# xl-tang3/RCOT

Hardware: AMD Instinct MI355X
Metric: 128x128 patches/sec (gen+critic step) (higher is better)
Workload: dtype fp32 (exact fp32 MFMA everywhere); 1 GPU; BASELINE configs[1]: Restormer T_net(decoder=True)+F_net(128), denoise_50, RMSprop, paired, B=8/GPU 128x128; global_batch=8, patch=128, parallelism=dp1, gemm_prec=fp32

## Files before the change

### include/rcot_hip.h

```cpp
#ifndef RCOT_HIP_H
#define RCOT_HIP_H
#include <stddef.h>

#ifdef __cplusplus
extern "C" {
#endif

#define RCOT_ABI_VERSION 26

#define RCOT_PREC_FP32 0
#define RCOT_PREC_BF16X3 1
#define RCOT_PREC_BF16X6 2
#define RCOT_PREC_BF16X1 3

int rcot_abi_version(void);
int rcot_debug_nt_coop(int mask);
int rcot_profile_begin(void);
int rcot_profile_end(char* out, int n);
int rcot_last_kernel(char* out, int n);

int rcot_conv1x1_fwd(const float* W, long ldw, const float* X, long sXb, float* Y, long sYb, int B, int Ci, int Co,
                     int N, const float* ln_mu, const float* ln_rs, const float* ln_w, const float* ln_b,
                     const float* R, long sRb, float beta, void* stream);
int rcot_conv1x1_dgrad(const float* W, long ldw, const float* dY, long sdYb, float* dX, long sdXb, int B, int Ci,
                       int Co, int N, float beta, void* stream);
int rcot_conv1x1_wgrad(const float* dY, long sdYb, const float* X, long sXb, float* dW, long ldw, int B, int Ci,
                       int Co, int N, const float* ln_mu, const float* ln_rs, const float* ln_w, const float* ln_b,
                       float beta, float* ws, size_t ws_bytes, int prec, void* stream);
int rcot_conv1x1_wgrad_slabs(const float* dY, long sdYb, const float* X, long sXb, int B, int Ci, int Co, int N,
                             const float* ln_mu, const float* ln_rs, const float* ln_w, const float* ln_b, float* ws,
                             size_t ws_bytes, int prec, int* S, int* ldws, void* stream);
// ... 47 lines not shown
int rcot_conv2d_dgrad(const float* dY, const float* Wt, float* dX, int B, int Ci, int H, int W, int Co, int KH,
                      int KW, int stride, int pad, float beta, const float* mask, float mslope, float* ws, size_t ws_bytes,
                      void* stream);
int rcot_conv2d_wgrad(const float* dY, const float* X, float* dWt, int B, int Ci, int H, int W, int Co, int KH,
                      int KW, int stride, int pad, float beta, float* ws, size_t ws_bytes, void* stream);
int rcot_conv_pcm_prep(const float* X, float* out, long ldo, int B, int C, int H, int W, int mode, void* stream);
int rcot_conv_pcm_wgrad(const float* dZp, const float* Xp, long ld, int N, int Wp, int Co, int Ci, float* dW, float beta, float* ws,
                        size_t ws_bytes, int prec, void* stream);
int rcot_conv_pcm_merge(const float* dQ, long ldq, float* dX, int B, int C, int H, int W, void* stream);
int rcot_conv_pcm_pack(const float* W, const int* rowoff, const int* koff, int M, int K, void* Apk, void* stream);
int rcot_conv_pcm(const void* Apk, int M, int K, const float* Xp, long ldb, int N, const int* tapoff, int ntaps, const float* bias,
                  float lrelu, const int* colmap, float* Y, long ldy, float* ws, size_t ws_bytes, void* stream);
int rcot_pixel_shuffle(const float* in, float* out, long planes, int H, int W, int mode, void* stream);

int rcot_ln_stats(const float* x, float* mu, float* rs, int B, int C, int N, void* stream);
int rcot_ln_bwd(const float* g, const float* x, const float* mu, const float* rs, const float* w, const float* dres,
                float* dx, float* dw, float* db, int B, int C, int N, void* ws, long ws_bytes, void* stream);
int rcot_ln_bwd_rows(int B, int C, int N);
int rcot_block_param_reduce(const float* part1, const float* part2, int rows, int C, float* gw1, float* gb1, float* gw2,
                            float* gb2, const float* dWo_part, float* gWo, const float* dtemp_part, float* gtemp, int B,
                            int heads, const long long* slab_sets, int n_sets, void* stream);

int rcot_dwconv3x3(const float* x, const float* w, float* y, int B, int C, int H, int W, int flip, void* stream);
int rcot_gdfn_gate_fwd(const float* p, const float* w, float* g, int B, int hid, int H, int W, void* stream);
int rcot_gdfn_gate_bwd(const float* p, const float* w, const float* dg, float* dd, float* dwg, int B, int hid, int H,
                       int W, void* stream);
int rcot_gdfn_bwd(const float* p, const float* w, const float* dg, float* dp, float* dwg, float* dd_scratch, int B, int hid,
                  int H, int W, void* stream);
int rcot_dwconv3x3_wgrad(const float* dy, const float* x, float* dw, int B, int C, int H, int W, void* stream);
int rcot_dwconv3x3_bwd(const float* dy, const float* x, const float* w, float* dx, float* dwg, int B, int C, int H, int W,
                       void* stream);

int rcot_row_sumsq(const float* x, float* out, int B, int R, int N, long sXb, void* stream);
int rcot_attn_softmax(const float* Graw, int S, int ld, const float* sq, const float* temp, float* Gn, float* A, int B,
                      int heads, int c, void* stream);
int rcot_attn_bwd_small(const float* dA, const float* A, const float* Gn, const float* sq, const float* temp,
                        float* dtemp_part, float* Eq, float* EqT, float* Dq, float* Dk, int B, int heads, int c,
                        void* stream);
int rcot_attn_bwd_fused(const float* dM, const float* Wo, const float* A, const float* Gn, const float* sq, const float* temp,
                        float* Mf, float* dWo_part, float* dtemp_part, float* Eq, float* EqT, float* Dq, float* Dk, int B,
                        int heads, int c, void* ws, long ws_bytes, void* stream);
int rcot_attn_core_fwd(const float* u, long sUb, const float* temp, const float* WoT, long ldwt, float* sq, float* Gn, float* A,
                       float* MfT, long ldm, long sMb, int B, int heads, int c, int N, float* ws, size_t ws_bytes, void* stream);
int rcot_attn_core_bwd(const float* dM, int S, int ldd, const float* Wo, const float* A, const float* Gn, const float* sq,
                       const float* temp, float* Mf, float* dWo_part, float* dtemp_part, float* Eq, float* EqT, float* Dq, float* Dk, int B,
                       int heads, int c, void* stream);
int rcot_batch_reduce(const float* src, float* dst, int B, long n, float beta, void* stream);

int rcot_lrelu_bwd(const float* dy, const float* a, float* dz, long n, float slope, void* stream);
int rcot_bias_grad(const float* dz, float* db, int B, int C, int P, void* stream);
int rcot_axpby2d(const float* x, long sx, const float* y, long sy, float* out, long so, long rows, long cols, float a,
                 float b, void* stream);
int rcot_fill(float* p, long n, float v, void* stream);
int rcot_lerp(const float* t, const float* f, const float* alpha, float* out, int B, long per, void* stream);
int rcot_gp_penalty(const float* g, float* norms, float* u0, float* gp_out, int B, long per, float inv_global_batch,
                    void* stream);

int rcot_ot_reduce(const float* degraded, const float* restored, const float* target, float* sums, int B, long per,
                   void* stream);
int rcot_fft_plan(int n, int* radices, int cap);
int rcot_ot_spectrum(const float* degraded, const float* restored, const int* de_id, float* gF, float* spec, float* ws,
                     size_t ws_bytes, int B, int H, int W, void* stream);
int rcot_ot_grad(const float* degraded, const float* restored, const float* target, const int* de_id, const float* gF,
                 const float* sums, const float* spec, float* dout, float* scal, int B, long per, float sigma,
                 float Sigma, long global_batch, void* stream);

// ... 28 lines not shown
```

### rcot_amd/csrc/attn_core.hip

```cpp
#include <cstdlib>
#include "common.h"
#include "../../include/rcot_hip.h"

using namespace rcot;

namespace {

typedef float f32x4 __attribute__((ext_vector_type(4)));

__device__ __forceinline__ float clamp_norm(float sumsq) { return fmaxf(sqrtf(sumsq), 1e-12f); }

template <int CT>
struct AC {
    static constexpr int cp = 16 * CT;
    static constexpr int c = CT == 2 ? 24 : cp;
    static constexpr int LDA = (cp % 32 == 16) ? cp : cp + 16;
    static constexpr int PX = CT == 6 ? 128 : 256;
    static constexpr int Q4 = PX / 4;
    static constexpr int LDQ = PX + 8;
    static constexpr int NW = CT == 6 ? 8 : 4;
    static constexpr int NT = 64 * NW;
    static constexpr int RPP = NT / Q4;
    static constexpr int KQ = cp / RPP;
    static constexpr int MTW = CT == 6 ? 1 : 2;
// ... 254 lines not shown
                const int i = wave + NW * r, j = lane + 64 * q;
                a[r][q] += (i < c && j < c) ? gp[(long)s * cc + i * c + j] : 0.f;
            }
    }
#pragma unroll
    for (int r = 0; r < NR; ++r)
#pragma unroll
        for (int q = 0; q < NJ; ++q) {
            const int i = wave + NW * r, j = lane + 64 * q;
            if (i < c && j < c) Gs[i * LDA + j] = a[r][q];
        }
    const float* sp = sqpart + z * S * 2 * c;
    for (int r = tid; r < 2 * c; r += NT) {
        float t = sp[r];
        for (int s = 1; s < S; ++s) t += sp[(long)s * 2 * c + r];
        sqs[r < c ? r : cp + r - c] = t;
        if (ms == 0) sq[(long)b * 2 * C + (r < c ? h * c + r : C + h * c + r - c)] = t;
    }
    __syncthreads();
    attn_tail<CT>(Gs, sqs, bfr, h, b, heads, temp, Gn, A, MfT, ldm, sMb, mt0, mt1, ms == 0);
}

template <int CT>
int launch_core_fwd(const float* u, long sUb, const float* temp, const float* WoT, long ldwt, float* sq, float* Gn, float* A, float* MfT,
                    long ldm, long sMb, int B, int heads, int c, int N, float* ws, size_t ws_bytes, hipStream_t st) {
    using K = AC<CT>;
    const int C = heads * c;
    static bool once = (hipFuncSetAttribute((const void*)qk_stats_kernel<CT>, hipFuncAttributeMaxDynamicSharedMemorySize, 160 * 1024) ==
                        hipSuccess);
    (void)once;
    const int ms = cdiv(C / 16, K::MT_WG);
    if (N == 256 && CT != 6) {
        RCOT_LAUNCH(qk_stats_kernel<CT>, dim3(ms, heads, B), dim3(K::NT), K::smem_stats, st, u, sUb, heads, N, N, nullptr,
                           nullptr, temp, WoT, ldwt, sq, Gn, A, MfT, ldm, sMb);
        RCOT_LAUNCH_CHECK();
        return RCOT_OK;
    }
    const int pxw = N == 256 ? 128 : (N > 16384 && N % 2048 == 0) ? 2048 : ((N > 1024 && N % 512 == 0) ? 512 : 256);
    const int S = N / pxw;
    const size_t Z = (size_t)B * heads;
    const size_t need = Z * S * ((size_t)c * c + 2 * c) * sizeof(float);
    if (!ws || ws_bytes < need) return RCOT_EWORKSPACE;
    float* gpart = ws;
    float* sqpart = ws + Z * S * c * c;
    RCOT_LAUNCH(qk_stats_kernel<CT>, dim3(S, heads, B), dim3(K::NT), K::smem_stats, st, u, sUb, heads, N, pxw, gpart, sqpart,
                       temp, WoT, ldwt, sq, Gn, A, MfT, ldm, sMb);
// ... 246 lines not shown
    RCOT_LAUNCH_CHECK();
    return RCOT_OK;
}

}

extern "C" {

int rcot_attn_core_fwd(const float* u, long sUb, const float* temp, const float* WoT, long ldwt, float* sq, float* Gn, float* A,
                       float* MfT, long ldm, long sMb, int B, int heads, int c, int N, float* ws, size_t ws_bytes, void* stream) {
    if (!u || !temp || !WoT || !sq || !Gn || !A || !MfT || B <= 0 || heads <= 0 || c <= 0 || N <= 0 || B > 65535 || heads > 65535)
        return RCOT_EINVAL;
    const int C = heads * c;
    if ((reinterpret_cast<uintptr_t>(u) & 15) || (sUb & 3) || ldwt < C || ldm < C) return RCOT_EINVAL;
    if ((C % 16) || (N % 256) || N > 65536) return RCOT_EUNSUPPORTED;
    if (N > 4096 && (N % 512)) return RCOT_EUNSUPPORTED;
    hipStream_t st = (hipStream_t)stream;
    if (c == 48) return launch_core_fwd<3>(u, sUb, temp, WoT, ldwt, sq, Gn, A, MfT, ldm, sMb, B, heads, c, N, ws, ws_bytes, st);
    if (c == 96) return launch_core_fwd<6>(u, sUb, temp, WoT, ldwt, sq, Gn, A, MfT, ldm, sMb, B, heads, c, N, ws, ws_bytes, st);
    if (c == 24) return launch_core_fwd<2>(u, sUb, temp, WoT, ldwt, sq, Gn, A, MfT, ldm, sMb, B, heads, c, N, ws, ws_bytes, st);
    return RCOT_EUNSUPPORTED;
}

int rcot_attn_core_bwd(const float* dM, int S, int ldd, const float* Wo, const float* A, const float* Gn, const float* sq,
                       const float* temp, float* Mf, float* dWo_part, float* dtemp_part, float* Eq, float* EqT, float* Dq, float* Dk, int B,
                       int heads, int c, void* stream) {
    if (!dM || !Wo || !A || !Gn || !sq || !temp || !Mf || !dWo_part || !dtemp_part || !Eq || !EqT || !Dq || !Dk || B <= 0 ||
        heads <= 0 || B > 65535 || heads > 65535 || S < 0 || S > 8)
        return RCOT_EINVAL;
    const int C = heads * c;
    if ((C % 16) || (c != 24 && c != 48 && c != 96)) return RCOT_EUNSUPPORTED;
    if (S == 0) ldd = C;
    if (ldd < C || (ldd & 3) || (reinterpret_cast<uintptr_t>(dM) & 15) || (reinterpret_cast<uintptr_t>(Wo) & 15)) return RCOT_EINVAL;
    const long sDs = (long)C * ldd, sDb = (long)(S < 1 ? 1 : S) * sDs;
    hipStream_t st = (hipStream_t)stream;
    if (c == 48) return launch_core_bwd<3>(dM, S, ldd, sDs, sDb, Wo, A, Gn, sq, temp, Mf, dWo_part, dtemp_part, Eq, EqT, Dq, Dk, B, heads, st);
    if (c == 96) return launch_core_bwd<6>(dM, S, ldd, sDs, sDb, Wo, A, Gn, sq, temp, Mf, dWo_part, dtemp_part, Eq, EqT, Dq, Dk, B, heads, st);
    return launch_core_bwd<2>(dM, S, ldd, sDs, sDb, Wo, A, Gn, sq, temp, Mf, dWo_part, dtemp_part, Eq, EqT, Dq, Dk, B, heads, st);
}

}
```

### rcot_amd/csrc/pointwise.hip

```cpp
#include <cstdlib>
#include "common.h"
#include "../../include/rcot_hip.h"

using namespace rcot;

namespace {

constexpr int LN_TX = 16, LN_TY = 16, LN_PIX = LN_TX * 4;

__device__ __forceinline__ float4 f4_add(float4 a, float4 b) { return make_float4(a.x + b.x, a.y + b.y, a.z + b.z, a.w + b.w); }

template <int TX>
__device__ __forceinline__ float4 reduce_rows(float4 v, float4* red, int tx, int ty) {
    constexpr int TY = 256 / TX;
    __syncthreads();
    red[ty * TX + tx] = v;
    __syncthreads();
    float4 t = red[tx];
#pragma unroll
    for (int i = 1; i < TY; ++i) t = f4_add(t, red[i * TX + tx]);
    return t;
}

__global__ __launch_bounds__(256) void ln_stats_kernel(const float* __restrict__ x, float* __restrict__ mu,
// ... 431 lines not shown
    b.plane = q / ((long)hq * wq);
    const int rem = (int)(q - b.plane * (long)hq * wq);
    const int ys = rem / wq;
    b.y0 = ys * 4;
    b.x0 = (rem - ys * wq) * 4;
    return b;
}

template <bool FLIP, bool NB>
__global__ __launch_bounds__(256) void dwconv_kernel(const float* __restrict__ x, const float* __restrict__ w,
                                                     float* __restrict__ y, long nblocks, int C, int H, int W) {
    const long q = (long)blockIdx.x * 256 + threadIdx.x;
    if (q >= nblocks) return;
    const BlockIdx4 b = block4(q, H, W);
    const int c = (int)(b.plane % C);
    Patch r;
    if (NB) load_patch_nb(x + b.plane * H * W, H, W, b.y0, b.x0, r);
    else load_patch(x + b.plane * H * W, H, W, b.y0, b.x0, r);
    float o[4][4];
    stencil16<FLIP>(r, w + c * 9, o);
    float* yp = y + b.plane * H * W + (long)b.y0 * W + b.x0;
#pragma unroll
    for (int i = 0; i < 4; ++i) *reinterpret_cast<float4*>(yp + (long)i * W) = make_float4(o[i][0], o[i][1], o[i][2], o[i][3]);
}

template <bool NB>
__global__ __launch_bounds__(256) void gate_fwd_kernel(const float* __restrict__ p, const float* __restrict__ w,
                                                       float* __restrict__ g, long nblocks, int hid, int H, int W) {
    const long q = (long)blockIdx.x * 256 + threadIdx.x;
    if (q >= nblocks) return;
    const BlockIdx4 b = block4(q, H, W);
    const long bi = b.plane / hid;
    const int j = (int)(b.plane - bi * hid);
    const long hw = (long)H * W;
    const float* p1 = p + (bi * 2 * hid + j) * hw;
    Patch r;
    float d1[4][4], d2[4][4];
    if (NB) {
        PatchRows q1, q2;
        patch_request(p1, H, W, b.y0, b.x0, q1);
        patch_request(p1 + (long)hid * hw, H, W, b.y0, b.x0, q2);
        patch_land(q1, H, W, b.y0, b.x0, r);
        stencil16<false>(r, w + j * 9, d1);
        patch_land(q2, H, W, b.y0, b.x0, r);
        stencil16<false>(r, w + (j + hid) * 9, d2);
    } else {
// ... 739 lines not shown
    RCOT_LAUNCH_CHECK();
    return RCOT_OK;
}

int rcot_dwconv3x3(const float* x, const float* w, float* y, int B, int C, int H, int W, int flip, void* stream) {
    if (!x || !w || !y || B <= 0 || C <= 0 || H <= 0 || W <= 0) return RCOT_EINVAL;
    if ((W & 3) || (H & 3)) {
        if (flip) return RCOT_EINVAL;
        const long total = (long)B * C * H * W;
        RCOT_LAUNCH(dwconv_any_kernel, dim3(grid_for(total)), dim3(256), 0, (hipStream_t)stream, x, w, y, total, C, H, W);
        RCOT_LAUNCH_CHECK();
        return RCOT_OK;
    }
    const long nq = (long)B * C * (H >> 2) * (W >> 2);
    const bool nb = nb_lanes_ok(W);
#define RCOT_DW(F, NB_) do { note_kernel("dwconv_kernel<%s, %s>", tf(F), tf(NB_)); RCOT_LAUNCH((dwconv_kernel<F, NB_>), dim3(cdiv(nq, 256)), dim3(256), 0, (hipStream_t)stream, x, w, y, nq, C, H, W); } while (0)
    if (flip) { if (nb) RCOT_DW(true, true); else RCOT_DW(true, false); }
    else { if (nb) RCOT_DW(false, true); else RCOT_DW(false, false); }
#undef RCOT_DW
    RCOT_LAUNCH_CHECK();
    return RCOT_OK;
}

int rcot_gdfn_gate_fwd(const float* p, const float* w, float* g, int B, int hid, int H, int W, void* stream) {
    if (!p || !w || !g || B <= 0 || hid <= 0 || H <= 0 || W <= 0) return RCOT_EINVAL;
    if ((W & 3) || (H & 3)) {
        const long total = (long)B * hid * H * W;
        RCOT_LAUNCH(gate_fwd_any_kernel, dim3(grid_for(total)), dim3(256), 0, (hipStream_t)stream, p, w, g, total, hid, H, W);
        RCOT_LAUNCH_CHECK();
        return RCOT_OK;
    }
    const long nq = (long)B * hid * (H >> 2) * (W >> 2);
    if (nb_lanes_ok(W))
        RCOT_LAUNCH(gate_fwd_kernel<true>, dim3(cdiv(nq, 256)), dim3(256), 0, (hipStream_t)stream, p, w, g, nq, hid, H, W);
    else
        RCOT_LAUNCH(gate_fwd_kernel<false>, dim3(cdiv(nq, 256)), dim3(256), 0, (hipStream_t)stream, p, w, g, nq, hid, H, W);
    RCOT_LAUNCH_CHECK();
    return RCOT_OK;
}

int rcot_gdfn_gate_bwd(const float* p, const float* w, const float* dg, float* dd, float* dwg, int B, int hid, int H,
                       int W, void* stream) {
    if (!p || !w || !dg || !dd || B <= 0 || hid <= 0 || H <= 0 || W <= 0 || (W & 3) || (H & 3)) return RCOT_EINVAL;
    const long cols = (long)B * hid * (W >> 2);
    bool fused = true;
    int rc;
// ... 128 lines not shown
```

### rcot_amd/lib.py

```python
from __future__ import annotations

import ctypes as C
import os

_HERE = os.path.dirname(os.path.abspath(__file__))
ABI_VERSION = 26
PREC_FP32, PREC_BF16X3, PREC_BF16X6, PREC_BF16X1 = 0, 1, 2, 3
LIB_PATH = os.environ.get("RCOT_LIB") or os.path.join(_HERE, "librcot_hip.so")


class RcotLibraryError(RuntimeError):
    pass


class RcotKernelError(RuntimeError):
    pass


_f = C.c_void_p
_l = C.c_long
_i = C.c_int
_fl = C.c_float
_d = C.c_double
_sz = C.c_size_t

class KmajorDesc(C.Structure):
    _fields_ = [("At", _f), ("lda", _l), ("sAo", _l), ("sAi", _l), ("a_rows", _i),
                ("Bm", _f), ("ldb", _l), ("sBo", _l), ("sBi", _l),
                ("C", _f), ("ldc", _l), ("sCo", _l), ("sCi", _l),
# ... 21 lines not shown
                         _f, _f, _l, _i, _f, _f, _f, _f, _f, _i, _i, _i, _i, _i, _fl, _f, _sz, _i, _f],
    "rcot_gemm_kmajor_stats": [_f, _l, _l, _l, _i, _f, _l, _l, _l, _f, _l, _l, _l, _f, _l, _l, _l, _f, _f, _l, _i, _i, _i, _i, _i, _f],
    "rcot_kmajor_desc_size": [],
    "rcot_gemm_kmajor_multi": [_f, _i, _i, _i, _f],
    "rcot_pack_weight": [_f, _l, _i, _i, _f, _f, _f, _f, _f, _f, _f, _f, _f, _f, _f, _f, _f],
    "rcot_pack_weights": [_f, _f, _i, _f],
    "rcot_linear_fwd": [_f, _f, _f, _f, _i, _i, _i, _fl, _f, _sz, _f],
    "rcot_linear_dgrad": [_f, _f, _f, _i, _i, _i, _f, _sz, _f],
    "rcot_linear_wgrad": [_f, _f, _f, _i, _i, _i, _fl, _f],
    "rcot_conv2d_fwd": [_f, _f, _f, _f, _i, _i, _i, _i, _i, _i, _i, _i, _i, _fl, _i, _f, _f, _fl, _f, _sz, _f],
    "rcot_conv2d_dgrad": [_f, _f, _f, _i, _i, _i, _i, _i, _i, _i, _i, _i, _fl, _f, _fl, _f, _sz, _f],
    "rcot_conv2d_wgrad": [_f, _f, _f, _i, _i, _i, _i, _i, _i, _i, _i, _i, _fl, _f, _sz, _f],
    "rcot_conv_pcm_prep": [_f, _f, _l, _i, _i, _i, _i, _i, _f],
    "rcot_conv_pcm_wgrad": [_f, _f, _l, _i, _i, _i, _i, _f, _fl, _f, _sz, _i, _f],
    "rcot_conv_pcm_merge": [_f, _l, _f, _i, _i, _i, _i, _f],
    "rcot_conv_pcm_pack": [_f, _f, _f, _i, _i, _f, _f],
    "rcot_conv_pcm": [_f, _i, _i, _f, _l, _i, _f, _i, _f, _fl, _f, _f, _l, _f, _sz, _f],
    "rcot_pixel_shuffle": [_f, _f, _l, _i, _i, _i, _f],
    "rcot_ln_stats": [_f, _f, _f, _i, _i, _i, _f],
    "rcot_ln_bwd": [_f, _f, _f, _f, _f, _f, _f, _f, _f, _i, _i, _i, _f, _l, _f],
    "rcot_ln_bwd_rows": [_i, _i, _i],
    "rcot_block_param_reduce": [_f, _f, _i, _i, _f, _f, _f, _f, _f, _f, _f, _f, _i, _i, _f, _i, _f],
    "rcot_dwconv3x3": [_f, _f, _f, _i, _i, _i, _i, _i, _f],
    "rcot_gdfn_gate_fwd": [_f, _f, _f, _i, _i, _i, _i, _f],
    "rcot_gdfn_gate_bwd": [_f, _f, _f, _f, _f, _i, _i, _i, _i, _f],
    "rcot_gdfn_bwd": [_f, _f, _f, _f, _f, _f, _i, _i, _i, _i, _f],
    "rcot_dwconv3x3_wgrad": [_f, _f, _f, _i, _i, _i, _i, _f],
    "rcot_dwconv3x3_bwd": [_f, _f, _f, _f, _f, _i, _i, _i, _i, _f],
    "rcot_row_sumsq": [_f, _f, _i, _i, _i, _l, _f],
    "rcot_attn_softmax": [_f, _i, _i, _f, _f, _f, _f, _i, _i, _i, _f],
    "rcot_attn_bwd_small": [_f, _f, _f, _f, _f, _f, _f, _f, _f, _f, _i, _i, _i, _f],
    "rcot_attn_bwd_fused": [_f] * 13 + [_i, _i, _i, _f, _l, _f],
    "rcot_attn_core_fwd": [_f, _l, _f, _f, _l, _f, _f, _f, _f, _l, _l, _i, _i, _i, _i, _f, _sz, _f],
    "rcot_attn_core_bwd": [_f, _i, _i] + [_f] * 12 + [_i, _i, _i, _f],
    "rcot_batch_reduce": [_f, _f, _i, _l, _fl, _f],
    "rcot_lrelu_bwd": [_f, _f, _f, _l, _fl, _f],
    "rcot_bias_grad": [_f, _f, _i, _i, _i, _f],
    "rcot_axpby2d": [_f, _l, _f, _l, _f, _l, _l, _l, _fl, _fl, _f],
    "rcot_fill": [_f, _l, _fl, _f],
    "rcot_lerp": [_f, _f, _f, _f, _i, _l, _f],
    "rcot_gp_penalty": [_f, _f, _f, _f, _i, _l, _fl, _f],
    "rcot_ot_reduce": [_f, _f, _f, _f, _i, _l, _f],
    "rcot_fft_plan": [_i, _f, _i],
    "rcot_ot_spectrum": [_f, _f, _f, _f, _f, _f, _sz, _i, _i, _i, _f],
    "rcot_ot_grad": [_f, _f, _f, _f, _f, _f, _f, _f, _f, _i, _l, _fl, _fl, _l, _f],
    "rcot_patch_prep": [_f, _f, _i, _i, _i, _i, _i, _i, _fl, C.c_ulonglong, _f, _f, _f],
    "rcot_rmsprop_step": [_f, _f, _f, _l, _d, _d, _d, _d, _f],
    "rcot_adam_step": [_f, _f, _f, _f, _l, _d, _d, _d, _d, _i, _d, _f],
    "rcot_prelu_fwd": [_f, _f, _f, _l, _f],
    "rcot_prelu_bwd": [_f, _f, _f, _f, _f, _l, _f, _sz, _f],
    "rcot_row_dot": [_f, _f, _f, _l, _i, _fl, _f],
    "rcot_row_scale_add": [_f, _f, _f, _f, _fl, _f, _l, _i, _f],
    "rcot_ca_gate_fwd": [_f, _f, _f, _f, _f, _i, _i, _i, _f],
    "rcot_ca_gate_bwd": [_f, _f, _f, _f, _f, _f, _f, _f, _f, _i, _i, _i, _f, _sz, _f],
    "rcot_bilinear_down2": [_f, _f, _l, _i, _i, _f],
    "rcot_bilinear_down2_bwd": [_f, _f, _l, _i, _i, _fl, _f],
# ... 48 lines not shown
```

### rcot_amd/net_restormer.py

```python
from __future__ import annotations

from collections import OrderedDict
from typing import Callable, Dict, List, Optional

import numpy as np

import torch

from . import params as P


class ParamStore:

    def __init__(self, be, shapes, live_order: List[str], dead: List[str]):
        self.be = be
        self.shapes = list(shapes)
        self.layout = P.make_layout(shapes, live_order, dead)
        self.flat = be.zeros(self.layout.n_total)
        self.grad = be.zeros(self.layout.n_total)
        self.p: Dict[str, torch.Tensor] = {}
        self.g: Dict[str, torch.Tensor] = {}
        for name, shp in self.shapes:
            o = self.layout.offset[name]
            n = int(np.prod(shp))
# ... 120 lines not shown
        B, C3, H, W = u.shape
        N = H * W
        uu = u.view(B, 3, self.heads, self.c, N)
        return uu[:, 0], uu[:, 1], u.view(B, 3, self.C, N)[:, 2].unsqueeze(1)

    def forward(self, x, save: bool, wmask: Optional[int] = None, in_stats=None, want_stats: bool = False):
        assert not (save and wmask is not None)
        be, C, hd, c, hid = self.be, self.C, self.heads, self.c, self.hid
        B, _, H, W = x.shape
        N = H * W
        fast = be.kmajor_worth(C, N, B)
        pstats = wmask is None and getattr(be, "stats_ok", None) is not None and be.stats_ok(C, N, B)
        self.out_stats = None
        t = be.empty(B, 3 * C, H, W)
        if in_stats is not None and pstats:
            mu1, rs1 = in_stats
            be.conv1x1_fwd(self.Wqkv, x, t, ln=(mu1, rs1, self.w1, self.b1), packed=self.pk_qkv)
        else:
            mu1, rs1 = be.empty(B, N), be.empty(B, N)
            be.conv1x1_fwd(self.Wqkv, x, t, ln=(mu1, rs1, self.w1, self.b1), packed=self.pk_qkv, ln_compute=True)
        if wmask is not None:
            t[..., wmask:].zero_()
        u = be.empty(B, 3 * C, H, W)
        be.dwconv3x3(t, self.Wdw, u)
        if wmask is not None:
            u[..., wmask:].zero_()
        sq = be.empty(B, 2 * C)
        Q, K, V = self._qkv_views(u)
        Gn, A, MfT = be.empty(B, hd, c, c), be.empty(B, hd, c, c), be.empty(B, C, C)
        if not be.attn_core_fwd(u, self.temp, self.pk_o[0], sq, Gn, A, MfT):
            be.row_sumsq(u[:, :2 * C], sq)
            Graw = be.bmm_nt_slabs(Q, K)
            if Graw is None:
                Graw = be.empty(B, hd, c, c)
                be.bmm_nt(Q, K, Graw)
            be.attn_softmax(Graw, sq, self.temp, Gn, A)
            be.bmm_nn(A, self._woT_heads(B), MfT.view(B, hd, c, C), transA=True)
        y = be.empty(B, C, H, W)
        mu2, rs2 = be.empty(B, N), be.empty(B, N)
        if fast and pstats:
            be.gemm_kmajor_stats(MfT.unsqueeze(1), V, y.view(B, 1, C, N), C, C, x.view(B, 1, C, N), (mu2, rs2))
        elif fast:
            be.gemm_kmajor(MfT.unsqueeze(1), V, y.view(B, 1, C, N), C, C, R=x.view(B, 1, C, N))
        else:
            be.bmm_nn(MfT.unsqueeze(1), V, y.view(B, 1, C, N), transA=True, R=x.view(B, 1, C, N))
        pp = be.empty(B, 2 * hid, H, W)
        be.conv1x1_fwd(self.Win, y, pp, ln=(mu2, rs2, self.w2, self.b2), packed=self.pk_in, ln_compute=not (fast and pstats))
        if wmask is not None:
            pp[..., wmask:].zero_()
        gg = be.empty(B, hid, H, W)
        be.gdfn_gate_fwd(pp, self.Wdw2, gg)
        out = be.empty(B, C, H, W)
        if want_stats and pstats and fast:
            self.out_stats = (be.empty(B, N), be.empty(B, N))
            be.conv1x1_fwd(self.Wout, gg, out, R=y, packed=self.pk_out, stats=self.out_stats)
        else:
            be.conv1x1_fwd(self.Wout, gg, out, R=y, packed=self.pk_out)
        ctx = (x, mu1, rs1, t, u, sq, Gn, A, y, mu2, rs2, pp, gg) if save else None
        return out, ctx

# ... 676 lines not shown
```

### rcot_amd/ops.py

```python
from __future__ import annotations

from typing import Optional, Sequence, Tuple

import os
import sys

import ctypes as C

import torch

from . import lib as _lib

LN = Optional[Tuple[torch.Tensor, torch.Tensor, torch.Tensor, torch.Tensor]]


ctypes_ll = C.c_longlong


def _ptr(t: Optional[torch.Tensor]):
    return None if t is None else t.data_ptr()


_raw_stream = getattr(torch._C, "_cuda_getCurrentRawStream", None) or (lambda i: torch.cuda.current_stream(i).cuda_stream)

# ... 58 lines not shown
    dev = torch.cuda.current_device() if torch.cuda.is_available() else -1
    if dev not in _DEFAULT:
        _DEFAULT[dev] = HipBackend()
    return _DEFAULT[dev]


class HipBackend:

    name = "hip"

    def __init__(self, device: Optional[torch.device] = None, workspace_bytes: int = 256 << 20):
        if not torch.cuda.is_available():
            raise _lib.RcotLibraryError("no HIP device visible: the RCOT hot path has no CPU fallback")
        self.L = _lib.load()
        self.device = torch.device("cuda", torch.cuda.current_device()) if device is None else torch.device(device)
        self._dev_index = self.device.index if self.device.index is not None else torch.cuda.current_device()
        self.ws = torch.empty(workspace_bytes // 4, dtype=torch.float32, device=self.device)
        self.ws_bytes = self.ws.numel() * 4
        self.prec = PREC_BY_NAME[os.environ.get("RCOT_GEMM_PREC", DEFAULT_PREC)]
        self._poison = os.environ.get("RCOT_POISON", "0") == "1"
        self.overlap = os.environ.get("RCOT_OVERLAP", "1") != "0"
        self._raw_events = os.environ.get("RCOT_RAW_EVENTS", "1") != "0"
        self.attn_core_maxn = 4096
        self.ln_fused = True
        self.prod_stats = True
        self._ev_ring, self._ev_next = [], -1
        self.x6_packs = self.prec == _lib.PREC_BF16X6
        self._side = torch.cuda.Stream(device=self.device) if self.overlap else None
        self._ws_side = torch.empty_like(self.ws) if self.overlap else None
        self._ws_slabs_gen = [torch.empty_like(self.ws), torch.empty_like(self.ws)]
        self._held = []
        self._pcm_cache = {}
        self._pcm_pinned = {}
        self._pcm_touched = set()
        self.pcm_pinning = False
        self._plan = None
        self._side_pending = False
        self._ln_scratch = [[torch.empty(1024 * 1024, dtype=torch.float32, device=self.device) for _ in range(2)] for _ in range(2)]
        self._ln_rows = 0
        self._gen = 0
        self._gen_event = [None, None]
        self._held_gen = [[], []]
        self._defer_close_env = os.environ.get("RCOT_DEFER_CLOSE")

    @property
    def defer_close(self):
# ... 703 lines not shown
                launch()
            if self._raw_events:
                ev, side = self._new_handover(), self._side.cuda_stream
                self._host(lambda: ev.record(side))
            else:
                ev = torch.cuda.Event()
                self._host(lambda: ev.record(self._side))
            self._gen_event[g] = ev
            self._held_gen[g] = self._held + [dWo_part, dtemp_part]
            self._held = []
            self._side_pending = True
            self._gen ^= 1
            return
        if close_block:
            self.side_join()
        launch()

    def dwconv3x3(self, x, w, y, flip: bool = False):
        B, Cc, H, W = x.shape
        assert x.is_contiguous() and y.is_contiguous() and w.is_contiguous()
        _lib.check(self.L.rcot_dwconv3x3(x.data_ptr(), w.data_ptr(), y.data_ptr(), B, Cc, H, W, int(flip), self._st()),
                   "rcot_dwconv3x3")

    def gdfn_gate_fwd(self, p, w, g):
        B, c2, H, W = p.shape
        assert p.is_contiguous() and g.is_contiguous() and w.is_contiguous()
        _lib.check(self.L.rcot_gdfn_gate_fwd(p.data_ptr(), w.data_ptr(), g.data_ptr(), B, c2 // 2, H, W, self._st()),
                   "rcot_gdfn_gate_fwd")

    def gdfn_gate_bwd(self, p, w, dg, dd, dw=None):
        B, c2, H, W = p.shape
        assert p.is_contiguous() and dg.is_contiguous() and dd.is_contiguous() and (dw is None or dw.is_contiguous())
        _lib.check(self.L.rcot_gdfn_gate_bwd(p.data_ptr(), w.data_ptr(), dg.data_ptr(), dd.data_ptr(), _ptr(dw), B, c2 // 2,
                                             H, W, self._st()), "rcot_gdfn_gate_bwd")

    @staticmethod
    def gdfn_bwd_needs_scratch(H: int, W: int) -> bool:
        wq = W // 4
        if wq > 64 or 64 % wq:
            return True
        for rs in (16, 8, 4):
            tpp = -(-H // rs) * wq
            if not (tpp % 256 == 0 or tpp % 64 == 0 or (tpp < 64 and tpp & (tpp - 1) == 0)):
                return True
        return False

# ... 12 lines not shown

    def dwconv3x3_wgrad(self, dy, x, dw):
        B, Cc, H, W = x.shape
        assert dy.is_contiguous() and x.is_contiguous() and dw.is_contiguous()
        _lib.check(self.L.rcot_dwconv3x3_wgrad(dy.data_ptr(), x.data_ptr(), dw.data_ptr(), B, Cc, H, W, self._st()),
                   "rcot_dwconv3x3_wgrad")

    def row_sumsq(self, x, out):
        B, R, N, sx = self._bcn(x, "row_sumsq x")
        assert out.is_contiguous()
        _lib.check(self.L.rcot_row_sumsq(x.data_ptr(), out.data_ptr(), B, R, N, sx, self._st()), "rcot_row_sumsq")

    def attn_softmax(self, Graw, sq, temp, Gn, A):
        B, heads, c, _ = Gn.shape
        for t in (sq, temp, Gn, A):
            assert t.is_contiguous()
        if isinstance(Graw, tuple):
            gp, S, ld = Graw
        else:
            assert Graw.is_contiguous() and tuple(Graw.shape) == tuple(Gn.shape)
            gp, S, ld = Graw.data_ptr(), 0, c
        _lib.check(self.L.rcot_attn_softmax(gp, S, ld, sq.data_ptr(), temp.data_ptr(), Gn.data_ptr(), A.data_ptr(),
                                            B, heads, c, self._st()), "rcot_attn_softmax")

    def attn_core_fwd(self, u, temp, WoT, sq, Gn, A, MfT) -> bool:
        B, heads, c, _ = Gn.shape
        N = u.shape[2] * u.shape[3]
        if N > self.attn_core_maxn:
            return False
        for t in (u, temp, sq, Gn, A, MfT):
            assert t.is_contiguous()
        assert WoT.stride(1) == 1 and tuple(MfT.shape) == (B, heads * c, heads * c) and u.shape[1] == 3 * heads * c
        rc = self.L.rcot_attn_core_fwd(u.data_ptr(), u.stride(0), temp.data_ptr(), WoT.data_ptr(), WoT.stride(0), sq.data_ptr(),
                                       Gn.data_ptr(), A.data_ptr(), MfT.data_ptr(), MfT.stride(1), MfT.stride(0), B, heads, c, N,
                                       self.ws.data_ptr(), self.ws_bytes, self._st())
        if rc == _lib.EUNSUPPORTED:
            return False
        _lib.check(rc, "rcot_attn_core_fwd")
        return True

    def attn_bwd_small(self, dA, A, Gn, sq, temp, dtemp_part, Eq, EqT, Dq, Dk):
        B, heads, c, _ = A.shape
        for t in (dA, A, Gn, sq, temp, dtemp_part, Eq, EqT, Dq, Dk):
            assert t.is_contiguous()
        _lib.check(self.L.rcot_attn_bwd_small(dA.data_ptr(), A.data_ptr(), Gn.data_ptr(), sq.data_ptr(), temp.data_ptr(),
                                              dtemp_part.data_ptr(), Eq.data_ptr(), EqT.data_ptr(), Dq.data_ptr(), Dk.data_ptr(), B, heads,
# ... 191 lines not shown
```

### rcot_amd/profiling.py

```python
from __future__ import annotations

import ctypes
from collections import defaultdict
from typing import Dict

import torch

GEMM_OPS = ("gemm_kmajor", "gemm_kmajor_stats", "gemm_kmajor_multi", "conv1x1_fwd", "conv1x1_dgrad", "conv1x1_dgrad_wgrad_slabs", "conv1x1_wgrad", "conv1x1_wgrad_slabs", "bmm_nn", "bmm_nt",
            "bmm_nt_slabs", "linear_fwd", "linear_dgrad",
            "linear_wgrad", "conv2d_fwd", "conv2d_dgrad", "conv2d_wgrad")
OTHER_OPS = ("ln_stats", "ln_bwd", "dwconv3x3", "gdfn_gate_fwd", "gdfn_gate_bwd", "gdfn_bwd", "dwconv3x3_wgrad", "dwconv3x3_bwd", "row_sumsq",
             "attn_softmax", "attn_bwd_small", "batch_reduce", "block_param_reduce", "lrelu_bwd", "bias_grad", "axpby", "fill", "lerp", "gp_penalty",
             "pixel_shuffle", "pack_weight", "ot_reduce", "ot_spectrum", "ot_grad", "rmsprop_step", "adam_step")


def _numel(t):
    if not isinstance(t, torch.Tensor):
        return 0
    n = 1
    for sz, st in zip(t.shape, t.stride()):
        if st != 0:
            n *= sz
    return n


def _flops(name, a, kw):
    if name == "conv1x1_dgrad_wgrad_slabs":
        return 4.0 * a[0].shape[0] * a[0].shape[1] * a[1].shape[0] * (a[1].numel() // (a[1].shape[0] * a[1].shape[1]))
    if name.startswith("conv1x1"):
        ts = [t for t in a[:3]]
        w = ts[0] if name not in ("conv1x1_wgrad", "conv1x1_wgrad_slabs") else ts[2]
        x = ts[1]
        return 2.0 * w.shape[0] * w.shape[1] * x.shape[0] * (x.numel() // (x.shape[0] * x.shape[1]))
    if name == "gemm_kmajor_multi":
# ... 154 lines not shown
```

Baseline: 105.8 patches/s.

## Fuse Q/K row sum-of-squares into dwconv and fold slab reduction into attention tail

For attention levels with c=48 and N above the core-fused threshold, the depthwise 3x3 conv now also emits per-workgroup partial sums of squares for the Q/K rows. This removes the separate row_sumsq pass over u. A new slab-fold kernel sums the split-K Gram slabs and the sq partials, then runs the existing attention tail (normalise, softmax, Wo fold) in one launch. That replaces the separate softmax and bmm_nn launches. The cost is an extra reduction epilogue with a __syncthreads in the conv kernel, plus a fold kernel that reads every slab.

```diff
diff --git a/include/rcot_hip.h b/include/rcot_hip.h
--- a/include/rcot_hip.h
+++ b/include/rcot_hip.h
@@ -6,7 +6,7 @@
 extern "C" {
 #endif
 
-#define RCOT_ABI_VERSION 26
+#define RCOT_ABI_VERSION 27
 
 #define RCOT_PREC_FP32 0
 #define RCOT_PREC_BF16X3 1
@@ -100,6 +100,8 @@
                             int heads, const long long* slab_sets, int n_sets, void* stream);
 
 int rcot_dwconv3x3(const float* x, const float* w, float* y, int B, int C, int H, int W, int flip, void* stream);
+int rcot_dwconv3x3_sq(const float* x, const float* w, float* y, float* sqpart, int sq_rows, int B, int C, int H, int W,
+                      void* stream);
 int rcot_gdfn_gate_fwd(const float* p, const float* w, float* g, int B, int hid, int H, int W, void* stream);
 int rcot_gdfn_gate_bwd(const float* p, const float* w, const float* dg, float* dd, float* dwg, int B, int hid, int H,
                        int W, void* stream);
@@ -120,6 +122,8 @@
                         int heads, int c, void* ws, long ws_bytes, void* stream);
 int rcot_attn_core_fwd(const float* u, long sUb, const float* temp, const float* WoT, long ldwt, float* sq, float* Gn, float* A,
                        float* MfT, long ldm, long sMb, int B, int heads, int c, int N, float* ws, size_t ws_bytes, void* stream);
+int rcot_attn_slab_fold(const float* gslab, int S, int ld, const float* sqpart, int P, const float* temp, const float* WoT, long ldwt,
+                        float* sq, float* Gn, float* A, float* MfT, long ldm, long sMb, int B, int heads, int c, void* stream);
 int rcot_attn_core_bwd(const float* dM, int S, int ldd, const float* Wo, const float* A, const float* Gn, const float* sq,
                        const float* temp, float* Mf, float* dWo_part, float* dtemp_part, float* Eq, float* EqT, float* Dq, float* Dk, int B,
                        int heads, int c, void* stream);
diff --git a/rcot_amd/csrc/attn_core.hip b/rcot_amd/csrc/attn_core.hip
--- a/rcot_amd/csrc/attn_core.hip
+++ b/rcot_amd/csrc/attn_core.hip
@@ -300,6 +300,88 @@
 }
 
 template <int CT>
+__global__ __launch_bounds__(AC<CT>::NT) void slab_fold_kernel(const float* __restrict__ gslab, int S, int ld,
+                                                               const float* __restrict__ sqpart, int P, int heads,
+                                                               const float* __restrict__ temp, const float* __restrict__ WoT, long ldwt,
+                                                               float* __restrict__ sq, float* __restrict__ Gn, float* __restrict__ A,
+                                                               float* __restrict__ MfT, long ldm, long sMb) {
+    using K = AC<CT>;
+    constexpr int cp = K::cp, c = K::c, LDA = K::LDA, NT = K::NT, C4 = c / 4, NPC = (c * C4 + NT - 1) / NT;
+    static_assert(c == cp, "the slab route serves c = 48 and 96 (no padding rows to clear)");
+    extern __shared__ __attribute__((aligned(16))) float sm[];
+    float* Gs = sm;
+    float* sqs = Gs + cp * LDA;
+    const int tid = threadIdx.x;
+    const int ms = blockIdx.x, h = blockIdx.y, b = blockIdx.z;
+    const int C = heads * c;
+    const int mt0 = ms * K::MT_WG, mt1 = min(C / 16, mt0 + K::MT_WG);
+    float bfr[K::MTW][cp / 4];
+    fold_prefetch<CT>(bfr, WoT, ldwt, h, mt0, mt1);
+    const long z = (long)b * heads + h;
+    const long slab = (long)c * ld;
+    const float* gp = gslab + z * S * slab;
+    int src[NPC], dst[NPC];
+    f32x4 acc[NPC][4];
+#pragma unroll
+    for (int k = 0; k < NPC; ++k) {
+        const int p = tid + NT * k;
+        const bool ok = p < c * C4;
+        const int i = ok ? p / C4 : 0, j = ok ? 4 * (p % C4) : 0;
+        src[k] = i * ld + j;
+        dst[k] = ok ? i * LDA + j : -1;
+#pragma unroll
+        for (int u = 0; u < 4; ++u) acc[k][u] = f32x4{0.f, 0.f, 0.f, 0.f};
+    }
+    int s = 0;
+#pragma unroll 1
+    for (; s + 4 <= S; s += 4) {
+        f32x4 v[NPC][4];
+#pragma unroll
+        for (int k = 0; k < NPC; ++k)
+#pragma unroll
+            for (int u = 0; u < 4; ++u) v[k][u] = *reinterpret_cast<const f32x4*>(gp + (long)(s + u) * slab + src[k]);
+#pragma unroll
+        for (int k = 0; k < NPC; ++k)
+#pragma unroll
+            for (int u = 0; u < 4; ++u) acc[k][u] += v[k][u];
+    }
+#pragma unroll 1
+    for (; s < S; ++s) {
+#pragma unroll
+        for (int k = 0; k < NPC; ++k) {
+            const f32x4 v = *reinterpret_cast<const f32x4*>(gp + (long)s * slab + src[k]);
+#pragma unroll
+            for (int u = 0; u < 4; ++u)
+                if ((s & 3) == u) acc[k][u] += v;
+        }
+    }
+#pragma unroll
+    for (int k = 0; k < NPC; ++k)
+        if (dst[k] >= 0) *reinterpret_cast<f32x4*>(Gs + dst[k]) = (acc[k][0] + acc[k][1]) + (acc[k][2] + acc[k][3]);
+    for (int r = tid; r < 2 * c; r += NT) {
+        const int row = r < c ? h * c + r : C + h * c + r - c;
+        const float* sp = sqpart + ((long)b * 2 * C + row) * P;
+        float t = sp[0];
+        for (int q = 1; q < P; ++q) t += sp[q];
+        sqs[r < c ? r : cp + r - c] = t;
+        if (ms == 0) sq[(long)b * 2 * C + row] = t;
+    }
+    __syncthreads();
+    attn_tail<CT>(Gs, sqs, bfr, h, b, heads, temp, Gn, A, MfT, ldm, sMb, mt0, mt1, ms == 0);
+}
+
+template <int CT>
+int launch_slab_fold(const float* gslab, int S, int ld, const float* sqpart, int P, const float* temp, const float* WoT, long ldwt,
+                     float* sq, float* Gn, float* A, float* MfT, long ldm, long sMb, int B, int heads, hipStream_t st) {
+    using K = AC<CT>;
+    const int ms = cdiv(heads * K::c / 16, K::MT_WG);
+    RCOT_LAUNCH(slab_fold_kernel<CT>, dim3(ms, heads, B), dim3(K::NT), K::smem_fold, st, gslab, S, ld, sqpart, P, heads, temp, WoT,
+                       ldwt, sq, Gn, A, MfT, ldm, sMb);
+    RCOT_LAUNCH_CHECK();
+    return RCOT_OK;
+}
+
+template <int CT>
 int launch_core_fwd(const float* u, long sUb, const float* temp, const float* WoT, long ldwt, float* sq, float* Gn, float* A, float* MfT,
                     long ldm, long sMb, int B, int heads, int c, int N, float* ws, size_t ws_bytes, hipStream_t st) {
     using K = AC<CT>;
@@ -592,6 +674,19 @@
     return RCOT_EUNSUPPORTED;
 }
 
+int rcot_attn_slab_fold(const float* gslab, int S, int ld, const float* sqpart, int P, const float* temp, const float* WoT, long ldwt,
+                        float* sq, float* Gn, float* A, float* MfT, long ldm, long sMb, int B, int heads, int c, void* stream) {
+    if (!gslab || !sqpart || !temp || !WoT || !sq || !Gn || !A || !MfT || S <= 0 || P <= 0 || B <= 0 || heads <= 0 || B > 65535 ||
+        heads > 65535)
+        return RCOT_EINVAL;
+    const int C = heads * c;
+    if (ld < c || (ld & 3) || (reinterpret_cast<uintptr_t>(gslab) & 15) || ldwt < C || ldm < C) return RCOT_EINVAL;
+    hipStream_t st = (hipStream_t)stream;
+    if (c == 48) return launch_slab_fold<3>(gslab, S, ld, sqpart, P, temp, WoT, ldwt, sq, Gn, A, MfT, ldm, sMb, B, heads, st);
+    if (c == 96) return launch_slab_fold<6>(gslab, S, ld, sqpart, P, temp, WoT, ldwt, sq, Gn, A, MfT, ldm, sMb, B, heads, st);
+    return RCOT_EUNSUPPORTED;
+}
+
 int rcot_attn_core_bwd(const float* dM, int S, int ldd, const float* Wo, const float* A, const float* Gn, const float* sq,
                        const float* temp, float* Mf, float* dWo_part, float* dtemp_part, float* Eq, float* EqT, float* Dq, float* Dk, int B,
                        int heads, int c, void* stream) {
diff --git a/rcot_amd/csrc/pointwise.hip b/rcot_amd/csrc/pointwise.hip
--- a/rcot_amd/csrc/pointwise.hip
+++ b/rcot_amd/csrc/pointwise.hip
@@ -477,6 +477,35 @@
     float* yp = y + b.plane * H * W + (long)b.y0 * W + b.x0;
 #pragma unroll
     for (int i = 0; i < 4; ++i) *reinterpret_cast<float4*>(yp + (long)i * W) = make_float4(o[i][0], o[i][1], o[i][2], o[i][3]);
+}
+
+template <bool NB>
+__global__ __launch_bounds__(256) void dwconv_sq_kernel(const float* __restrict__ x, const float* __restrict__ w,
+                                                        float* __restrict__ y, float* __restrict__ sqpart, int sq_rows, int parts,
+                                                        int C, int H, int W) {
+    __shared__ float red[4];
+    const long q = (long)blockIdx.x * 256 + threadIdx.x;
+    const BlockIdx4 b = block4(q, H, W);
+    const int c = (int)(b.plane % C);
+    Patch r;
+    if (NB) load_patch_nb(x + b.plane * H * W, H, W, b.y0, b.x0, r);
+    else load_patch(x + b.plane * H * W, H, W, b.y0, b.x0, r);
+    float o[4][4];
+    stencil16<false>(r, w + c * 9, o);
+    float* yp = y + b.plane * H * W + (long)b.y0 * W + b.x0;
+#pragma unroll
+    for (int i = 0; i < 4; ++i) *reinterpret_cast<float4*>(yp + (long)i * W) = make_float4(o[i][0], o[i][1], o[i][2], o[i][3]);
+    if (c >= sq_rows) return;
+    float a = 0.f;
+#pragma unroll
+    for (int i = 0; i < 4; ++i) a += (o[i][0] * o[i][0] + o[i][1] * o[i][1]) + (o[i][2] * o[i][2] + o[i][3] * o[i][3]);
+    a = wave_sum(a);
+    if ((threadIdx.x & 63) == 0) red[threadIdx.x >> 6] = a;
+    __syncthreads();
+    if (threadIdx.x == 0) {
+        const long img = b.plane / C;
+        sqpart[(img * sq_rows + c) * parts + blockIdx.x % parts] = (red[0] + red[1]) + (red[2] + red[3]);
+    }
 }
 
 template <bool NB>
@@ -1262,6 +1291,25 @@
     return RCOT_OK;
 }
 
+int rcot_dwconv3x3_sq(const float* x, const float* w, float* y, float* sqpart, int sq_rows, int B, int C, int H, int W,
+                      void* stream) {
+    if (!x || !w || !y || !sqpart || B <= 0 || C <= 0 || H <= 0 || W <= 0 || sq_rows <= 0 || sq_rows > C) return RCOT_EINVAL;
+    const long per = (long)(H >> 2) * (W >> 2);
+    if ((W & 3) || (H & 3) || (per & 255)) return RCOT_EUNSUPPORTED;
+    const int parts = (int)(per >> 8);
+    const long nwg = (long)B * C * parts;
+    if (nwg > 0x7fffffffL) return RCOT_EUNSUPPORTED;
+    if (nb_lanes_ok(W)) {
+        note_kernel("dwconv_sq_kernel<true>");
+        RCOT_LAUNCH(dwconv_sq_kernel<true>, dim3((unsigned)nwg), dim3(256), 0, (hipStream_t)stream, x, w, y, sqpart, sq_rows, parts, C, H, W);
+    } else {
+        note_kernel("dwconv_sq_kernel<false>");
+        RCOT_LAUNCH(dwconv_sq_kernel<false>, dim3((unsigned)nwg), dim3(256), 0, (hipStream_t)stream, x, w, y, sqpart, sq_rows, parts, C, H, W);
+    }
+    RCOT_LAUNCH_CHECK();
+    return RCOT_OK;
+}
+
 int rcot_gdfn_gate_fwd(const float* p, const float* w, float* g, int B, int hid, int H, int W, void* stream) {
     if (!p || !w || !g || B <= 0 || hid <= 0 || H <= 0 || W <= 0) return RCOT_EINVAL;
     if ((W & 3) || (H & 3)) {
diff --git a/rcot_amd/lib.py b/rcot_amd/lib.py
--- a/rcot_amd/lib.py
+++ b/rcot_amd/lib.py
@@ -4,7 +4,7 @@
 import os
 
 _HERE = os.path.dirname(os.path.abspath(__file__))
-ABI_VERSION = 26
+ABI_VERSION = 27
 PREC_FP32, PREC_BF16X3, PREC_BF16X6, PREC_BF16X1 = 0, 1, 2, 3
 LIB_PATH = os.environ.get("RCOT_LIB") or os.path.join(_HERE, "librcot_hip.so")
 
@@ -72,6 +72,7 @@
     "rcot_ln_bwd_rows": [_i, _i, _i],
     "rcot_block_param_reduce": [_f, _f, _i, _i, _f, _f, _f, _f, _f, _f, _f, _f, _i, _i, _f, _i, _f],
     "rcot_dwconv3x3": [_f, _f, _f, _i, _i, _i, _i, _i, _f],
+    "rcot_dwconv3x3_sq": [_f, _f, _f, _f, _i, _i, _i, _i, _i, _f],
     "rcot_gdfn_gate_fwd": [_f, _f, _f, _i, _i, _i, _i, _f],
     "rcot_gdfn_gate_bwd": [_f, _f, _f, _f, _f, _i, _i, _i, _i, _f],
     "rcot_gdfn_bwd": [_f, _f, _f, _f, _f, _f, _i, _i, _i, _i, _f],
@@ -82,6 +83,7 @@
     "rcot_attn_bwd_small": [_f, _f, _f, _f, _f, _f, _f, _f, _f, _f, _i, _i, _i, _f],
     "rcot_attn_bwd_fused": [_f] * 13 + [_i, _i, _i, _f, _l, _f],
     "rcot_attn_core_fwd": [_f, _l, _f, _f, _l, _f, _f, _f, _f, _l, _l, _i, _i, _i, _i, _f, _sz, _f],
+    "rcot_attn_slab_fold": [_f, _i, _i, _f, _i, _f, _f, _l, _f, _f, _f, _f, _l, _l, _i, _i, _i, _f],
     "rcot_attn_core_bwd": [_f, _i, _i] + [_f] * 12 + [_i, _i, _i, _f],
     "rcot_batch_reduce": [_f, _f, _i, _l, _fl, _f],
     "rcot_lrelu_bwd": [_f, _f, _f, _l, _fl, _f],
diff --git a/rcot_amd/net_restormer.py b/rcot_amd/net_restormer.py
--- a/rcot_amd/net_restormer.py
+++ b/rcot_amd/net_restormer.py
@@ -166,20 +166,25 @@
         if wmask is not None:
             t[..., wmask:].zero_()
         u = be.empty(B, 3 * C, H, W)
-        be.dwconv3x3(t, self.Wdw, u)
+        sqp = None
+        if getattr(be, "attn_slab_tail", False) and wmask is None and N > be.attn_core_maxn and c in be.slab_tail_widths:
+            sqp = be.dwconv3x3_sq(t, self.Wdw, u, 2 * C)
+        if sqp is None:
+            be.dwconv3x3(t, self.Wdw, u)
         if wmask is not None:
             u[..., wmask:].zero_()
         sq = be.empty(B, 2 * C)
         Q, K, V = self._qkv_views(u)
         Gn, A, MfT = be.empty(B, hd, c, c), be.empty(B, hd, c, c), be.empty(B, C, C)
         if not be.attn_core_fwd(u, self.temp, self.pk_o[0], sq, Gn, A, MfT):
-            be.row_sumsq(u[:, :2 * C], sq)
             Graw = be.bmm_nt_slabs(Q, K)
-            if Graw is None:
-                Graw = be.empty(B, hd, c, c)
-                be.bmm_nt(Q, K, Graw)
-            be.attn_softmax(Graw, sq, self.temp, Gn, A)
-            be.bmm_nn(A, self._woT_heads(B), MfT.view(B, hd, c, C), transA=True)
+            if not (sqp is not None and Graw is not None and be.attn_slab_fold(Graw, sqp, self.temp, self.pk_o[0], sq, Gn, A, MfT)):
+                be.row_sumsq(u[:, :2 * C], sq)
+                if Graw is None:
+                    Graw = be.empty(B, hd, c, c)
+                    be.bmm_nt(Q, K, Graw)
+                be.attn_softmax(Graw, sq, self.temp, Gn, A)
+                be.bmm_nn(A, self._woT_heads(B), MfT.view(B, hd, c, C), transA=True)
         y = be.empty(B, C, H, W)
         mu2, rs2 = be.empty(B, N), be.empty(B, N)
         if fast and pstats:
diff --git a/rcot_amd/ops.py b/rcot_amd/ops.py
--- a/rcot_amd/ops.py
+++ b/rcot_amd/ops.py
@@ -104,6 +104,8 @@
         self.overlap = os.environ.get("RCOT_OVERLAP", "1") != "0"
         self._raw_events = os.environ.get("RCOT_RAW_EVENTS", "1") != "0"
         self.attn_core_maxn = 4096
+        self.attn_slab_tail = os.environ.get("RCOT_ATTN_SLAB_FOLD", "1") != "0"
+        self.slab_tail_widths = (48,)
         self.ln_fused = True
         self.prod_stats = True
         self._ev_ring, self._ev_next = [], -1
@@ -853,6 +855,19 @@
         _lib.check(self.L.rcot_dwconv3x3(x.data_ptr(), w.data_ptr(), y.data_ptr(), B, Cc, H, W, int(flip), self._st()),
                    "rcot_dwconv3x3")
 
+    def dwconv3x3_sq(self, x, w, y, sq_rows: int):
+        B, Cc, H, W = x.shape
+        assert x.is_contiguous() and y.is_contiguous() and w.is_contiguous()
+        per = (H // 4) * (W // 4)
+        if H % 4 or W % 4 or per % 256:
+            return None
+        part = self.empty(B, sq_rows, per // 256)
+        rc = self.L.rcot_dwconv3x3_sq(x.data_ptr(), w.data_ptr(), y.data_ptr(), part.data_ptr(), sq_rows, B, Cc, H, W, self._st())
+        if rc == _lib.EUNSUPPORTED:
+            return None
+        _lib.check(rc, "rcot_dwconv3x3_sq")
+        return part
+
     def gdfn_gate_fwd(self, p, w, g):
         B, c2, H, W = p.shape
         assert p.is_contiguous() and g.is_contiguous() and w.is_contiguous()
@@ -911,6 +926,19 @@
             gp, S, ld = Graw.data_ptr(), 0, c
         _lib.check(self.L.rcot_attn_softmax(gp, S, ld, sq.data_ptr(), temp.data_ptr(), Gn.data_ptr(), A.data_ptr(),
                                             B, heads, c, self._st()), "rcot_attn_softmax")
+
+    def attn_slab_fold(self, Graw, sqpart, temp, WoT, sq, Gn, A, MfT) -> bool:
+        B, heads, c, _ = Gn.shape
+        gp, S, ld = Graw
+        for t in (sqpart, temp, sq, Gn, A, MfT):
+            assert t.is_contiguous()
+        assert WoT.stride(1) == 1 and tuple(MfT.shape) == (B, heads * c, heads * c) and tuple(sqpart.shape[:2]) == (B, 2 * heads * c)
+        if c not in (48, 96):
+            return False
+        _lib.check(self.L.rcot_attn_slab_fold(gp, S, ld, sqpart.data_ptr(), sqpart.shape[2], temp.data_ptr(), WoT.data_ptr(), WoT.stride(0),
+                                              sq.data_ptr(), Gn.data_ptr(), A.data_ptr(), MfT.data_ptr(), MfT.stride(1), MfT.stride(0), B,
+                                              heads, c, self._st()), "rcot_attn_slab_fold")
+        return True
 
     def attn_core_fwd(self, u, temp, WoT, sq, Gn, A, MfT) -> bool:
         B, heads, c, _ = Gn.shape
diff --git a/rcot_amd/profiling.py b/rcot_amd/profiling.py
--- a/rcot_amd/profiling.py
+++ b/rcot_amd/profiling.py
@@ -9,7 +9,7 @@
 GEMM_OPS = ("gemm_kmajor", "gemm_kmajor_stats", "gemm_kmajor_multi", "conv1x1_fwd", "conv1x1_dgrad", "conv1x1_dgrad_wgrad_slabs", "conv1x1_wgrad", "conv1x1_wgrad_slabs", "bmm_nn", "bmm_nt",
             "bmm_nt_slabs", "linear_fwd", "linear_dgrad",
             "linear_wgrad", "conv2d_fwd", "conv2d_dgrad", "conv2d_wgrad")
-OTHER_OPS = ("ln_stats", "ln_bwd", "dwconv3x3", "gdfn_gate_fwd", "gdfn_gate_bwd", "gdfn_bwd", "dwconv3x3_wgrad", "dwconv3x3_bwd", "row_sumsq",
+OTHER_OPS = ("ln_stats", "ln_bwd", "dwconv3x3", "dwconv3x3_sq", "gdfn_gate_fwd", "gdfn_gate_bwd", "gdfn_bwd", "dwconv3x3_wgrad", "dwconv3x3_bwd", "row_sumsq",
              "attn_softmax", "attn_bwd_small", "batch_reduce", "block_param_reduce", "lrelu_bwd", "bias_grad", "axpby", "fill", "lerp", "gp_penalty",
              "pixel_shuffle", "pack_weight", "ot_reduce", "ot_spectrum", "ot_grad", "rmsprop_step", "adam_step")
 
```

Result: no change. 105.8 patches/s, median of 2 (-0.0%).
